# drdeford/FlipComplexityEmpirical

Measured on AMD Instinct MI355X. Metric: flip steps/sec (whole node), 100×100 grid k=4 batched chains; % HBM peak, higher is better.
Workload: dtype int32

## Files before the change

flipcomplexityempirical_amd/csrc/fw_grid16.hip:

```cpp
#include <hip/hip_runtime.h>

#include <cstdio>
#include <cstdlib>

#include <algorithm>

#include "fw_device.h"

#ifdef FW_STAMPS
__device__ unsigned long long g_stamps[16];
__device__ unsigned long long g_unit_t[2 * 65536];
__device__ unsigned long long g_unit_hw[65536];
#define UNIT_TIME(u, e)                                                         \
  do {                                                                          \
    uint64_t t_;                                                                \
    asm volatile("s_memrealtime %0\n\ts_waitcnt lgkmcnt(0)" : "=s"(t_)::"memory"); \
    if (__lane_id() == 0 && (u) < 65536) {                                      \
      g_unit_t[2 * (u) + (e)] = t_;                                             \
      if ((e) == 0)                                                             \
        g_unit_hw[u] = (unsigned long long)__builtin_amdgcn_s_getreg((31 << 11) | 4) | \
                       ((unsigned long long)__builtin_amdgcn_s_getreg((31 << 11) | 20) << 32); \
    }                                                                           \
  } while (0)
#define STAMP_DECL uint64_t st_acc[16] = {}; uint64_t st_t0 = 0;
// ... 7 lines not shown
    st_t0 = st_t1;                                            \
  } while (0)
#define STAMP_FLUSH                                           \
  if (__lane_id() == 0)                                       \
    for (int i_ = 0; i_ < 16; ++i_) atomicAdd(&g_stamps[i_], (unsigned long long)st_acc[i_]);
#define STAMP_COUNT(i, v) st_acc[i] += (uint64_t)(v)
#else
#define STAMP_COUNT(i, v)
#define STAMP_DECL
#define STAMP(i)
#define STAMP_FLUSH
#define UNIT_TIME(u, e)
#endif

#include <cstddef>

static_assert(sizeof(fw_chain_stats) == 136, "fw_chain_stats layout");
static_assert(offsetof(fw_chain_stats, yields) == 88 && offsetof(fw_chain_stats, sum_invb) == 112 &&
                  offsetof(fw_chain_stats, cut) == 120 && offsetof(fw_chain_stats, npairs) == 128,
              "fw_chain_stats layout");

#define HIST_ADD(ptr, v) atomicAdd(ptr, v)

void* fw_grid16_pick_lean(int lb, int mode, int G);
void* fw_grid16_pick_w2(int mode, int G);

namespace {

constexpr int ROW = 16;
constexpr int MAX_NW = 4;
constexpr uint32_t SCR_BLOCK = 15;
constexpr int LDS_GUARD = 16;

struct Hood16 {
  int x;
  uint32_t lx;
  uint32_t bits;
  uint32_t cnt;
  bool has_v;
  int deg;
};

struct GDiv {
  uint32_t m, s;
  __device__ __forceinline__ int operator()(int x) const {
    return (int)(__umul24((uint32_t)x, m) >> s);
  }
};
// ... 74 lines not shown
__device__ __forceinline__ uint32_t bsum4(uint32_t v) {
  return (v & 0xFFu) + ((v >> 8) & 0xFFu) + ((v >> 16) & 0xFFu) + (v >> 24);
}

__device__ __forceinline__ uint32_t spread4(uint32_t u) {
  const uint32_t t = ((u << 12) | u) & 0x000F000Fu;
  return ((t << 6) | t) & 0x03030303u;
}
__device__ __forceinline__ uint32_t onehot4(uint32_t s) {
  return __builtin_amdgcn_perm(0u, 0x08040201u, s);
}
__device__ __forceinline__ uint32_t low_bytes(int t) {
  const uint32_t tc = (uint32_t)min(max(t, 0), 4);
  return tc == 4u ? 0xFFFFFFFFu : (1u << (8u * tc)) - 1u;
}
__device__ __forceinline__ uint32_t ne_bytes(uint32_t a, uint32_t b) {
  return ~((a & b) + 0x7F7F7F7Fu) & 0x80808080u;
}
__device__ __forceinline__ uint32_t byte_popc(uint32_t f) {
  const uint32_t t = f - ((f >> 1) & 0x55555555u);
  return (t & 0x33333333u) + ((t >> 2) & 0x33333333u);
}

template <int MODE, bool NEED_CD, bool BATCH = true>
__device__ __forceinline__ void weights4_swar(const LDS uint8_t* lab, int x0, int W, int H, int n,
                                              GDiv gd, uint32_t& w4, uint32_t& cd4) {
  w4 = 0;
  cd4 = 0;
  const int xs = x0 < n ? x0 : 0;
  const bool hasU = xs + 3 - W >= 0, hasD = xs + W < n;
  const LDS uint32_t* lw32 = reinterpret_cast<const LDS uint32_t*>(lab);
  const int xw[3] = {xs, hasU ? xs - W : xs, hasD ? xs + W : xs};
  uint32_t wlo[3], whi[3];
  int wbit[3];
#pragma unroll
  for (int t = 0; t < 3; ++t) {
    wbit[t] = (xw[t] - 1) * 2;
    const int wi = wbit[t] >> 5;
    wlo[t] = lw32[wi];
    whi[t] = lw32[wi + 1];
  }
  const int r0 = gd(x0);
  const int c0 = x0 - mulW(r0, W);
  const int tw = W - c0;
  const uint32_t t8 = (uint32_t)min(tw, 4) << 3;
  const uint32_t nxt = (uint32_t)(~0ull << t8);
  const uint32_t mN = low_bytes(n - x0);
  const uint32_t mU = r0 > 0 ? 0xFFFFFFFFu : nxt;
  const uint32_t mD = r0 < H - 2 ? 0xFFFFFFFFu : (r0 == H - 2 ? ~nxt : 0u);
  const uint32_t mL = ~((uint32_t)(0xFFull << t8) | (c0 == 0 ? 0xFFu : 0u));
  const uint32_t mR = ~(uint32_t)(0xFFull << (((uint32_t)min(tw, 5) << 3) - 8u));
  if constexpr (BATCH) __builtin_amdgcn_sched_barrier(0);
  uint32_t win[3];
#pragma unroll
  for (int t = 0; t < 3; ++t) {
    const int wi = wbit[t] >> 5;
    const uint64_t both = ((uint64_t)whi[t] << 32) | (wi >= 0 ? wlo[t] : 0u);
    win[t] = (uint32_t)(both >> (uint32_t)(wbit[t] - wi * 32)) & 0xFFFu;
  }
  const uint32_t own = win[0];
  const uint32_t up = hasU ? win[1] : 0u, dn = hasD ? win[2] : 0u;
  const uint32_t o_lo = onehot4(spread4(own)), o_hi = onehot4(spread4(own >> 8));
  const uint32_t L = o_lo;
  const uint32_t O = __builtin_amdgcn_alignbyte(o_hi, o_lo, 1);
  const uint32_t R = __builtin_amdgcn_alignbyte(o_hi, o_lo, 2);
  const uint32_t U = onehot4(spread4(up >> 2)), Dn = onehot4(spread4(dn >> 2));
  if constexpr (MODE != FW_PROPOSE_CUTEDGE) {
    const uint32_t bits = (U & mU) | (L & mL) | (R & mR) | (Dn & mD);
    w4 = byte_popc(bits & ~O & mN);
  }
  if constexpr (NEED_CD || MODE == FW_PROPOSE_CUTEDGE) {
    const uint32_t ne = (ne_bytes(U, O) & mU) >> 7, nl = (ne_bytes(L, O) & mL) >> 7,
                   nr = (ne_bytes(R, O) & mR) >> 7, nd = (ne_bytes(Dn, O) & mD) >> 7;
    cd4 = (ne + nl + nr + nd) & mN;
    if constexpr (MODE == FW_PROPOSE_CUTEDGE) w4 = cd4;
  }
}

template <int LB, int MODE, bool NEED_CD, bool BATCH = true>
__device__ __forceinline__ void weights4x(const LDS uint8_t* lab, int x0, int W, int H, int n,
                                          GDiv gd, uint32_t& w4, uint32_t& cd4) {
  if constexpr (LB == 2)
    weights4_swar<MODE, NEED_CD, BATCH>(lab, x0, W, H, n, gd, w4, cd4);
  else
    weights4<LB, MODE>(lab, x0, W, H, n, gd, w4, cd4);
}

__device__ __forceinline__ uint32_t bsum4m(uint32_t v) { return (v * 0x01010101u) >> 24; }


__device__ __forceinline__ int window_verdict8(uint64_t A, int q, int row, bool need, uint32_t& nflood) {
#ifdef FW_STAMPS
#define FLOOD_COUNT ++nflood
#else
#define FLOOD_COUNT
#endif
  constexpr uint64_t BORDER = 0x7Full | (0x7Full << 48) | 0x0001010101010101ull | 0x0040404040404040ull;
  const uint64_t src = A & ((1ull << 19) | (1ull << 26) | (1ull << 28) | (1ull << 35));
  const int sb = q == 0 ? 19 : q == 1 ? 26 : q == 2 ? 28 : 35;
  uint64_t x = (need && q < 4) ? src & (1ull << sb) : 0ull;
  if (x) {
    for (;;) {
      const uint64_t y = (x | (x << 1) | (x >> 1) | (x << 8) | (x >> 8)) & A;
      x = (y | (y << 1) | (y >> 1) | (y << 8) | (y >> 8)) & A;
      FLOOD_COUNT;
      if (x == y) break;
// ... 226 lines not shown
    lb = le;
    le = nl;
    rep = ballot(lane < m && (__ffsll((unsigned long long)cls) - 1) == lane);
    if (__popcll(rep) == 1) {
      verdict = 1;
      break;
    }
    const bool closed = lane < m && ((rep >> lane) & 1ull) && ((cls & pushed_src) == 0ull);
    if (ballot(closed)) {
      verdict = 0;
      break;
    }
  }
  bfs_deg += wave_sum(my_deg);
  for (int base = 0; base < nl; base += WAVE) {
    const int idx = base + lane;
    if (idx < nl) scr_clear(scr, (int)list_get(idx));
  }
  if (lane == 0) scr_clear(scr, v);
  lds_order();
  return verdict == 1;
}

template <int LB, int MODE, int PER, bool FULL, bool BIG, int R, bool W2 = false>
__device__ __forceinline__ void grid16_body(const FwRunParams& p) {
  static_assert(PER % 2 == 0, "group sums are read as u16 pairs");
  static_assert(R == 1 || R == 2 || R == 4, "rows per chain");
  static_assert(R == 1 || (!FULL && !BIG), "speculation: lean small-grid kernels only");
  constexpr int CPW = 4 / R;
  extern __shared__ __align__(16) uint8_t smem[];
  __shared__ int32_t s_lock;
  using P = PK<LB>;
  const int lane = __lane_id(), row = lane >> 4, q = lane & 15;
  const int sx = row & (R - 1);
  const int grp = row / R;
  const int gb = grp * R * ROW;
  const bool owner = sx == 0;
  const int wv = (int)(threadIdx.x >> 6);
  const int W = (int)in_vgpr((uint32_t)p.g.gw), H = (int)in_vgpr((uint32_t)p.g.gh);
  const int n = (int)in_vgpr((uint32_t)p.g.n);
  const int D = (int)in_vgpr((uint32_t)p.g.maxdeg), G = (int)in_vgpr((uint32_t)p.G);
  const int k = (int)in_vgpr((uint32_t)p.k);
  LDS uint8_t* const sm = (LDS uint8_t*)smem;
  LDS uint8_t* const lab = sm + LDS_GUARD + (wv * CPW + grp) * p.slot_stride;
  LDS uint32_t* const gsum = reinterpret_cast<LDS uint32_t*>(lab + p.off_gsum);
  LDS uint32_t* const ssum = reinterpret_cast<LDS uint32_t*>(lab + p.off_ssum);
  LDS uint32_t* const lvl1 = BIG ? ssum : gsum;
  LDS uint8_t* const scr = sm + p.off_scr;
// ... 66 lines not shown
      LDS u32x4* dst = reinterpret_cast<LDS u32x4*>(lab);
      const int nv = cached ? p.lab_copy16 : p.lab_bytes / 16;
      for (int i = sx * ROW + ql; i < nv; i += R * ROW) dst[i] = src[i];
    }
    int32_t pops = ql < k ? (int32_t)p.pops[(size_t)cc * k + ql] : 0;
    double thr_l = FULL && ql < 2 * D + 1 ? p.thr[(size_t)cc * p.thr_stride + ql] : 0.0;
    uint64_t thr53_l = ql < 2 * D + 1 ? p.thr53[(size_t)cc * p.thr_stride + ql] : 0ull;
    fw_chain_stats* stp = p.stats + cc;
    const uint64_t acc0 = FULL && p.sched ? stp->accepts : 0ull;
    auto sched_row = [&](uint64_t nacc) {
      const int64_t t = (int64_t)(acc0 + nacc) + 1 - p.sched_t0;
      const int64_t r = t < 0 ? 0 : (t >= p.sched_rows ? p.sched_rows - 1 : t);
      if (q < 2 * D + 1) {
        thr_l = p.sched[r * (2 * D + 1) + q];
        thr53_l = p.sched53[r * (2 * D + 1) + q];
      }
    };
    if (FULL && p.sched) sched_row(0);
    uint64_t att0 = stp->attempts;
    const bool first = has && !stp->stuck && stp->yields == 0 && att0 == 0;
    uint32_t n_att = 0;
    const uint64_t yields0 = stp->yields;
    int32_t stuck = has ? stp->stuck : 1;
    int64_t sum_cut = stp->sum_cut, sum_bnodes = stp->sum_bnodes;
    double sum_invb = stp->sum_invb;
    const bool waits_on = FULL && p.wsamp != nullptr;
    double wsum = waits_on ? p.wsamp[2 * (size_t)cc] : 0.0;
    double wcur = waits_on ? p.wsamp[2 * (size_t)cc + 1] : 0.0;
    uint32_t n_steps = 0, n_acc = 0, n_popf = 0, n_conf = 0, n_sdeg = 0, n_adeg = 0, n_bchg = 0;
    uint32_t retries = 0;
    uint64_t n_bfs = 0, n_bfsn = 0, n_bfsd = 0;
    uint32_t bpos_w = ROW * R;
    Pend pend = maps_on ? pend_load(p, cc) : Pend{-1, 0, 0u};
    int32_t bcnt = rule == FW_ACCEPT_BOUNDARY && ql < k ? p.bcnt[(size_t)cc * k + ql] : 0;
    lds_order();

    int32_t cut, bnodes, npairs;
    {
      uint32_t cut2 = 0, bn = 0, np = 0;
      for (int t2 = 0; t2 < (cached ? 0 : GW); ++t2) {
        uint32_t tot[2];
#pragma unroll
        for (int h = 0; h < 2; ++h) {
          uint32_t w4, cd4;
          weights4x<LB, MODE, true>(lab, (2 * t2 + h) * 64 + q * 4, W, H, n, gd, w4, cd4);
          const uint32_t ws = bsum4m(w4);
          cut2 += bsum4m(cd4);
          bn += ((cd4 & 0xFFu) != 0) + ((cd4 & 0xFF00u) != 0) + ((cd4 & 0xFF0000u) != 0) +
                ((cd4 & 0xFF000000u) != 0);
          np += ws;
          tot[h] = row_sum(ws);
        }
        if (q == 0 && has) gsum[t2] = tot[0] | (tot[1] << 16);
      }
      if constexpr (BIG) {
        for (int t2 = GW + q; t2 < SG * 8; t2 += ROW)
          if (has) gsum[t2] = 0u;
        lds_order();
        for (int w2 = q; w2 < 8 * PER; w2 += ROW) {
          uint32_t s2[2] = {0u, 0u};
#pragma unroll
          for (int h = 0; h < 2; ++h) {
            const int sg = 2 * w2 + h;
            if (sg < SG)
              for (int i = 0; i < 8; ++i) {
                const uint32_t g2 = gsum[sg * 8 + i];
                s2[h] += (g2 & 0xFFFFu) + (g2 >> 16);
              }
// ... 22 lines not shown
      int f = -1, sc = -1;
      for (int b0 = 0; b0 < RN; b0 += ROW) {
        const int r = b0 + q;
        const int ri = r < RN ? r : 0;
        uint32_t m = rowbits(ballot(r < RN && P::get(lab, p.ring_u[ri]) != P::get(lab, p.ring_w[ri])),
                             row);
        if (m && f < 0) {
          f = b0 + __ffs(m) - 1;
          m &= m - 1;
        }
        if (m && sc < 0) sc = b0 + __ffs(m) - 1;
      }
      return sc >= 0 ? f * RN + sc : RN * RN;
    };
    int32_t rpair = RN && has ? ring_pair() : 0;
    uint32_t rrun = 0;

    uint32_t hc0 = 0, hc1 = 0, hb0 = 0, hb1 = 0;
    int32_t base_c = max(0, cut - 16), base_b = max(0, bnodes - 16);
    auto observe = [&](bool on) {
      if (!on) return;
      if (FULL) rrun += 1;
      if (waits_on) wsum += wcur;
      sum_cut += cut;
      sum_bnodes += bnodes;
      sum_invb += invb;
      int ic = cut - base_c;
      if (ic < 0 || ic >= 2 * ROW) {
        if (hc0) HIST_ADD(p.hist_cut + base_c + q, (unsigned long long)hc0);
        if (hc1) HIST_ADD(p.hist_cut + base_c + ROW + q, (unsigned long long)hc1);
        hc0 = hc1 = 0;
        base_c = max(0, cut - ROW);
        ic = cut - base_c;
      }
      hc0 += ic == q;
      hc1 += ic == q + ROW;
      int ib = bnodes - base_b;
      if (ib < 0 || ib >= 2 * ROW) {
        if (hb0) HIST_ADD(p.hist_b + base_b + q, (unsigned long long)hb0);
        if (hb1) HIST_ADD(p.hist_b + base_b + ROW + q, (unsigned long long)hb1);
        hb0 = hb1 = 0;
        base_b = max(0, bnodes - ROW);
        ib = bnodes - base_b;
      }
      hb0 += ib == q;
      hb1 += ib == q + ROW;
    };
    if (waits_on && first) wcur = wait_draw(p.seed, FW_WAIT_T0, gid, p.wlp[bnodes]);
    observe(first && owner);

    U4 pb = {0u, 0u, 0u, 0u};
    int bpos = ROW;

    const bool unit_pop = !FULL || p.g.pop == nullptr;
    const uint32_t psh = (uint32_t)p.prio_shift;
    const uint32_t pstep = ustep >= (2u << psh) ? ustep >> psh : 2u;
    uint32_t pnext = pstep, plev = 0;
    if (psh == 3u && (__builtin_amdgcn_s_getreg((3 << 11) | 4) & 1u) == 0u) plev = 1;
    if (plev == 0) __builtin_amdgcn_s_setprio(3);
    else __builtin_amdgcn_s_setprio(2);
    for (;;) {
      STAMP(-1);
      if (!stuck && (retries >= (uint32_t)p.max_retries || npairs == 0)) stuck = 1;
      const bool act = has && !stuck && n_steps < ustep;
      if (ballot(act) == 0ull) break;
      if (rfl(n_steps) >= pnext) {
        pnext += pstep;
        plev = (plev + 1u) & 3u;
        if (plev == 0) __builtin_amdgcn_s_setprio(3);
        else if (plev == 1) __builtin_amdgcn_s_setprio(2);
        else if (plev == 2) __builtin_amdgcn_s_setprio(1);
        else __builtin_amdgcn_s_setprio(0);
      }

      U4 x;
      if constexpr (R == 1) {
        if (bpos == ROW) {
          if (n_sdeg >= p.fold_at) {
            if (q == 0 && has) {
              stp->pop_fail += n_popf;
              stp->contig_fail += n_conf;
              stp->sum_deg += n_sdeg;
            }
            att0 += n_att;
            n_att = n_popf = n_conf = n_sdeg = 0;
          }
          const uint64_t t = att0 + (uint64_t)(n_att + (uint32_t)q);
          pb = philox((uint32_t)t, (uint32_t)(t >> 32), (uint32_t)gid, (uint32_t)(gid >> 32),
                      in_vgpr(key0), in_vgpr(key1));
          bpos = 0;
        }
        x = U4{row_first(pb.x0), row_first(pb.x1), row_first(pb.x2), row_first(pb.x3)};
        pb = U4{row_shl1(pb.x0), row_shl1(pb.x1), row_shl1(pb.x2), row_shl1(pb.x3)};
        ++bpos;
        n_att += act ? 1u : 0u;
      } else {
        if (bpos_w > (uint32_t)(ROW * R - R)) {
          if (4u * n_att >= p.fold_at) {
            const uint32_t f0 = grp_sum<R>(n_popf, gb, q), f1 = grp_sum<R>(n_conf, gb, q);
            const uint32_t f2 = grp_sum<R>(n_sdeg, gb, q);
            if (q == 0 && owner && has) {
              stp->pop_fail += f0;
              stp->contig_fail += f1;
              stp->sum_deg += f2;
            }
            att0 += n_att;
            n_att = n_popf = n_conf = n_sdeg = 0;
          }
          const uint64_t t = att0 + (uint64_t)(n_att + (uint32_t)(sx * ROW + q));
          pb = philox((uint32_t)t, (uint32_t)(t >> 32), (uint32_t)gid, (uint32_t)(gid >> 32),
                      in_vgpr(key0), in_vgpr(key1));
          bpos_w = 0;
        }
        const int srcl = gb + (int)bpos_w + sx;
        x = U4{lane_read(pb.x0, srcl), lane_read(pb.x1, srcl), lane_read(pb.x2, srcl),
               lane_read(pb.x3, srcl)};
      }
      const uint32_t r = scale64(x.x0, x.x1, (uint32_t)(npairs > 0 ? npairs : 1));

      STAMP(0);
      uint32_t w2[PER / 2];
      uint32_t s = 0;
#pragma unroll
      for (int t = 0; t < PER / 2; ++t) {
        w2[t] = lvl1[q * (PER / 2) + t];
        s += (w2[t] & 0xFFFFu) + (w2[t] >> 16);
      }
      uint32_t pp[PER / 2];
      {
        uint32_t base = 0;
#pragma unroll
        for (int t = 0; t < PER / 2; ++t) {
          pp[t] = __umul24(base, 0x10001u) + (w2[t] + (w2[t] << 16));
          base = pp[t] >> 16;
        }
      }
      const uint32_t incl = row_scan(s);
      const uint32_t rb1 = rowbits(ballot(incl > r), row);
      const int Lw = __ffs(rb1) - 1;
      const uint32_t rl = r - (incl - s);
      typedef uint16_t u16x2 __attribute__((ext_vector_type(2)));
      const u16x2 rl2 = __builtin_bit_cast(u16x2, __umul24(rl & 0xFFFFu, 0x10001u));
      u16x2 mn = {0xFFFFu, 0xFFFFu}, wraps = {0u, 0u};
#pragma unroll
      for (int t = 0; t < PER / 2; ++t) {
        const u16x2 e = rl2 - __builtin_bit_cast(u16x2, pp[t]);
        mn = __builtin_elementwise_min(mn, e);
        wraps += e >> (uint16_t)15;
      }
      const uint32_t rem = min(rl, (uint32_t)min(mn.x, mn.y));
// ... 3 lines not shown
      int gi;
      uint32_t r1;
      uint32_t rbg = 1u;
      if constexpr (BIG) {
        const int sgi = min((int)(pk1 >> 16), SG - 1);
        const uint32_t r1s = pk1 & 0xFFFFu;
        const uint32_t g2 = gsum[sgi * 8 + (q >> 1)];
        const uint32_t gv = (q & 1) ? (g2 >> 16) : (g2 & 0xFFFFu);
        const uint32_t incg = row_scan(gv);
        rbg = rowbits(ballot(incg > r1s), row);
        const int Lg = __ffs(rbg) - 1;
        const uint32_t pkg =
            row_pick(((uint32_t)(sgi * 16 + q) << 16) | ((r1s - (incg - gv)) & 0xFFFFu), Lg, q);
        gi = min((int)(pkg >> 16), G - 1);
        r1 = pkg & 0xFFFFu;
      } else {
        gi = min((int)(pk1 >> 16), G - 1);
        r1 = pk1 & 0xFFFFu;
      }

      STAMP(1);
      const int x0 = gi * 64 + q * 4;
      uint32_t w4, cd4;
      weights4x<LB, MODE, false, !W2>(lab, x0, W, H, n, gd, w4, cd4);
      const uint32_t pref1 = w4 + (w4 << 8);
      const uint32_t pref = pref1 + (pref1 << 16);
      const uint32_t ws = pref >> 24;
      const uint32_t incl2 = row_scan(ws);
      const uint32_t rb2 = rowbits(ballot(incl2 > r1), row);
      const int L2 = __ffs(rb2) - 1;
      const uint32_t r2 = min(r1 - (incl2 - ws), 127u);
      const uint32_t gt = ((pref | 0x80808080u) - __builtin_amdgcn_perm(0u, r2 + 1u, 0u)) & 0x80808080u;
      const int t2 = gt ? (__ffs(gt) - 1) >> 3 : 3;
      const uint32_t bef2 = t2 ? (pref >> (8 * t2 - 8)) & 0xFFu : 0u;
      const uint32_t pk2 = row_pick(((uint32_t)(q * 4 + t2) << 16) | ((r2 - bef2) & 0xFFFFu), L2, q);
      const int v = min(gi * 64 + (int)(pk2 >> 16), n - 1);
      const uint32_t j = pk2 & 0xFFFFu;
      if (R == 1 && act && (rb1 == 0 || rb2 == 0 || rbg == 0)) stuck = 2;
      const bool go = act && rb1 != 0 && rb2 != 0 && rbg != 0;

      STAMP(2);
      int vr, vc;
      divmod(v, vr, vc);
      const int dv = (vr > 0) + (vc > 0) + (vc < W - 1) + (vr < H - 1);
      Hood16 h;
      h.x = -1;
      h.lx = NOLAB;
// ... 290 lines not shown
          }
        }
        if (sx < (int)cons) {
          n_sdeg += (uint32_t)dv;
          if (!pop_ok) n_popf += 1;
          else if (!contig) n_conf += 1;
          n_bfs += it_bfs;
          n_bfsn += it_bfsn;
          n_bfsd += it_bfsd;
        }
        n_steps = ns;
        retries = rt;
        n_att += cons;
        bpos_w += cons;
        const bool commit_me = sx == fpos;
        if (commit_me) {
          n_acc += 1;
          n_adeg += (uint32_t)dv;
          n_bchg += (uint32_t)(plus + minus);
          if (q == 0) P::axor(lab, v, a ^ d);
          if (mine && wn != wo) lds_add(gsum + (h.x >> 7), (wn - wo) << (16 * ((h.x >> 6) & 1)));
        }
        lds_order();
        uint32_t dl = commit_me && mine ? wn - wo : 0u;
        dl += (uint32_t)__builtin_amdgcn_update_dpp(0, (int)dl, 0x111, 0xF, 0xF, true);
        dl += (uint32_t)__builtin_amdgcn_update_dpp(0, (int)dl, 0x112, 0xF, 0xF, true);
        dl += (uint32_t)__builtin_amdgcn_update_dpp(0, (int)dl, 0x114, 0xF, 0xF, true);
        const int dnp = (int)(uint32_t)__builtin_amdgcn_update_dpp(0, (int)dl, 0x154, 0xF, 0xF, false);
        const int fsrc = gb + (fpos < 0 ? 0 : fpos) * ROW + q;
        const uint32_t pk = (uint32_t)(dcut + 8) | ((uint32_t)plus << 4) | ((uint32_t)minus << 8) |
                            (a << 12) | (d << 16) | ((uint32_t)(dnp + 64) << 20);
        const uint32_t pkf = lane_read(pk, fsrc);
        const uint64_t ib = (uint64_t)__double_as_longlong(invb_new);
        const uint32_t ibl = lane_read((uint32_t)ib, fsrc), ibh = lane_read((uint32_t)(ib >> 32), fsrc);
        for (uint32_t i = 0; i < kold; ++i) observe(owner);
        if (fpos >= 0) {
          npairs += (int)((pkf >> 20) & 127u) - 64;
          cut += (int)(pkf & 15u) - 8;
          bnodes += (int)((pkf >> 4) & 15u) - (int)((pkf >> 8) & 15u);
          invb = __longlong_as_double((long long)(((uint64_t)ibh << 32) | ibl));
          if ((uint32_t)q == ((pkf >> 12) & 15u)) pops -= 1;
          if ((uint32_t)q == ((pkf >> 16) & 15u)) pops += 1;
          observe(owner);
        }
        STAMP(5);
        continue;
// ... 24 lines not shown
        p.trace[(size_t)c * p.steps + n_steps] = accepted ? v * 64 + (int)d : -1;
      n_steps += valid ? 1u : 0u;
      if (maps_on && accepted) {
        const int64_t t = (int64_t)(yields0 + (n_steps - 1u) + (first ? 1u : 0u));
        if (q >= 1 && q <= 4 && h.x >= 0 && (h.lx == a || h.lx == d)) {
          const int e = q == 1   ? grid_eid_down(vr - 1, vc, W, H)
                        : q == 2 ? grid_eid_right(vr, vc - 1, W, H)
                        : q == 3 ? grid_eid_right(vr, vc, W, H)
                                 : grid_eid_down(vr, vc, W, H);
          map_edge(p, c, e, h.lx == a, t);
        }
        if (q == 0) map_run_end(p, c, pend, t);
        pend = Pend{v, (int32_t)d, (uint32_t)t};
      }

      if (accepted) {
        if (q == 0) P::axor(lab, v, a ^ d);
        if (mine && wn != wo) {
          lds_add(gsum + (h.x >> 7), (wn - wo) << (16 * ((h.x >> 6) & 1)));
          if (BIG) lds_add(ssum + (h.x >> 11), (wn - wo) << (16 * ((h.x >> 10) & 1)));
        }
      }
      lds_order();
      uint32_t dl = accepted && mine ? wn - wo : 0u;
      dl += (uint32_t)__builtin_amdgcn_update_dpp(0, (int)dl, 0x111, 0xF, 0xF, true);
      dl += (uint32_t)__builtin_amdgcn_update_dpp(0, (int)dl, 0x112, 0xF, 0xF, true);
      dl += (uint32_t)__builtin_amdgcn_update_dpp(0, (int)dl, 0x114, 0xF, 0xF, true);
      const int dnp = (int)(uint32_t)__builtin_amdgcn_update_dpp(0, (int)dl, 0x154, 0xF, 0xF, false);
      if (FULL && RN && accepted && p.ring_node[v]) {
        const int32_t np2 = ring_pair();
        if (np2 != rpair) {
          if (q == 0 && rrun) atomicAdd(p.hist_ring + rpair, (unsigned long long)rrun);
          rrun = 0;
          rpair = np2;
        }
      }
      STAMP(9);
      asm volatile("" ::"v"(invb_new));
      invb = accepted ? invb_new : invb;
      if (accepted) {
        n_acc += 1;
        if (FULL && p.sched) sched_row(n_acc);
        n_adeg += (uint32_t)dv;
        npairs += dnp;
        cut += dcut;
        bnodes += plus - minus;
// ... 35 lines not shown
      for (int i = qw; i < p.lab_copy16; i += ROW) dst[i] = src[i];
      if (qw < k) p.pops[(size_t)c * k + qw] = (int64_t)pops;
      if (qw < k && rule == FW_ACCEPT_BOUNDARY) p.bcnt[(size_t)c * k + qw] = bcnt;
      if (q == 0 && maps_on) pend_store(p, c, pend);
      if (q == 0 && waits_on) {
        p.wsamp[2 * (size_t)c] = wsum;
        p.wsamp[2 * (size_t)c + 1] = wcur;
      }
      if (q <= 8) {
        int qr = qw;
        if constexpr (!OPQ) asm volatile("" : "+v"(qr));
        uint64_t* rec = reinterpret_cast<uint64_t*>(stp) + 2 * qr;
        const uint64_t o0 = rec[0];
        const uint64_t o1 = qr < 8 ? rec[1] : 0ull;
        const uint64_t yinc = (uint64_t)n_steps + (first ? 1u : 0u);
        uint64_t w0, w1;
        switch (q) {
          case 0: w0 = att0 + n_att; w1 = o1 + n_steps; break;
          case 1: w0 = o0 + n_acc; w1 = o1 + n_popf; break;
          case 2: w0 = o0 + n_conf; w1 = o1 + n_bfs; break;
          case 3: w0 = o0 + n_bfsn; w1 = o1 + n_bfsd; break;
          case 4: w0 = o0 + n_sdeg; w1 = o1 + n_adeg; break;
          case 5: w0 = o0 + n_bchg; w1 = o1 + yinc; break;
          case 6: w0 = (uint64_t)sum_cut; w1 = (uint64_t)sum_bnodes; break;
          case 7:
            w0 = (uint64_t)__double_as_longlong(sum_invb);
            w1 = (uint64_t)(uint32_t)cut | ((uint64_t)(uint32_t)bnodes << 32);
            break;
          default: w0 = (uint64_t)(uint32_t)npairs | ((uint64_t)(uint32_t)stuck << 32); w1 = 0;
        }
        if (qr < 8) {
          typedef uint64_t u64x2 __attribute__((ext_vector_type(2)));
          *reinterpret_cast<u64x2*>(rec) = u64x2{w0, w1};
        } else {
          rec[0] = w0;
        }
      }
    }
    lds_order();
    UNIT_TIME(u, 1);
    if (seg + 1 < p.slices) {
      __builtin_amdgcn_fence(__ATOMIC_RELEASE, "agent");
      __hip_atomic_store(p.seg_done + quad, seg + 1, __ATOMIC_RELAXED, __HIP_MEMORY_SCOPE_AGENT);
    }
  }
  STAMP_FLUSH
}

template <int LB, int MODE, int PER, bool FULL, bool BIG>
__global__ __launch_bounds__(64 * MAX_NW) __attribute__((amdgpu_waves_per_eu(3))) void fw_grid16_kernel(FwRunParams p) {
  static_assert(!FULL, "FULL instantiations: fw_grid16_full_kernel");
  grid16_body<LB, MODE, PER, FULL, BIG, 1>(p);
}
template <int LB, int MODE, int PER, bool FULL, bool BIG>
__global__ __launch_bounds__(64 * MAX_NW) void fw_grid16_full_kernel(FwRunParams p) {
  grid16_body<LB, MODE, PER, true, BIG, 1>(p);
}
template <int LB, int MODE, int PER>
__global__ __launch_bounds__(64 * MAX_NW) void fw_grid16_w2_kernel(FwRunParams p) {
  grid16_body<LB, MODE, PER, false, false, 1, true>(p);
}

#ifndef FW_SPEC_WPE
#define FW_SPEC_WPE 3
#endif
template <int LB, int MODE, int PER, int R>
__global__ __launch_bounds__(64 * MAX_NW) __attribute__((amdgpu_waves_per_eu(FW_SPEC_WPE))) void
fw_grid16_spec_kernel(FwRunParams p) {
  grid16_body<LB, MODE, PER, false, false, R>(p);
}

int per16(int G) { return G <= 16 * 2 ? 2 : G <= 16 * 4 ? 4 : G <= 16 * 10 ? 10 : 16; }
int per16_big(int G) { return (G + 15) / 16 <= 32 ? 2 : 4; }
bool is_big(int G) { return G > 16 * 16; }

template <int LB, int MODE, int PER, bool FULL, bool BIG>
void* k16() {
  if constexpr (FULL)
    return reinterpret_cast<void*>(&fw_grid16_full_kernel<LB, MODE, PER, true, BIG>);
  else
    return reinterpret_cast<void*>(&fw_grid16_kernel<LB, MODE, PER, false, BIG>);
}

template <int LB, int MODE>
void* pick16_small_lean(int G) {
  switch (per16(G)) {
    case 2: return k16<LB, MODE, 2, false, false>();
    case 4: return k16<LB, MODE, 4, false, false>();
    case 10: return k16<LB, MODE, 10, false, false>();
    default: return k16<LB, MODE, 16, false, false>();
  }
}

template <int LB, int MODE, bool FULL>
void* pick16(int G) {
  if (is_big(G)) {
    if constexpr (LB == 4) {
      return nullptr;
    } else {
      return per16_big(G) == 2
                 ? k16<LB, MODE, 2, FULL, true>()
                 : k16<LB, MODE, 4, FULL, true>();
    }
  }
  if constexpr (LB == 3) {
    return nullptr;
  } else if constexpr (FULL) {
    switch (per16(G)) {
      case 2: return k16<LB, MODE, 2, true, false>();
      case 4: return k16<LB, MODE, 4, true, false>();
      case 10: return k16<LB, MODE, 10, true, false>();
      default: return k16<LB, MODE, 16, true, false>();
    }
  } else {
#if defined(FW_STAMPS)
    return pick16_small_lean<LB, MODE>(G);
#else
    return fw_grid16_pick_lean(LB, MODE, G);
#endif
  }
}

template <int MODE>
void* pick16_w2(int G) {
  if (is_big(G)) return nullptr;
  switch (per16(G)) {
    case 2: return reinterpret_cast<void*>(&fw_grid16_w2_kernel<2, MODE, 2>);
    case 4: return reinterpret_cast<void*>(&fw_grid16_w2_kernel<2, MODE, 4>);
    case 10: return reinterpret_cast<void*>(&fw_grid16_w2_kernel<2, MODE, 10>);
    default: return reinterpret_cast<void*>(&fw_grid16_w2_kernel<2, MODE, 16>);
  }
}

template <int LB, int MODE, int R>
void* pick16_spec(int G) {
  if (is_big(G) || LB == 3) return nullptr;
  switch (per16(G)) {
    case 2: return reinterpret_cast<void*>(&fw_grid16_spec_kernel<LB, MODE, 2, R>);
    case 4: return reinterpret_cast<void*>(&fw_grid16_spec_kernel<LB, MODE, 4, R>);
    case 10: return reinterpret_cast<void*>(&fw_grid16_spec_kernel<LB, MODE, 10, R>);
    default: return reinterpret_cast<void*>(&fw_grid16_spec_kernel<LB, MODE, 16, R>);
  }
}

template <int R>
void* pick16_spec_mode(const FwRunParams& p) {
  const bool cut = p.mode == FW_PROPOSE_CUTEDGE;
  if (p.lb == 2)
    return cut ? pick16_spec<2, FW_PROPOSE_CUTEDGE, R>(p.G) : pick16_spec<2, FW_PROPOSE_PAIRS, R>(p.G);
  if (p.lb == 4)
    return cut ? pick16_spec<4, FW_PROPOSE_CUTEDGE, R>(p.G) : pick16_spec<4, FW_PROPOSE_PAIRS, R>(p.G);
  return nullptr;
}

template <bool FULL>
void* pick16_mode(const FwRunParams& p) {
  const bool cut = p.mode == FW_PROPOSE_CUTEDGE;
  if (p.lb == 2)
    return cut ? pick16<2, FW_PROPOSE_CUTEDGE, FULL>(p.G) : pick16<2, FW_PROPOSE_PAIRS, FULL>(p.G);
  if (p.lb == 3)
    return cut ? pick16<3, FW_PROPOSE_CUTEDGE, FULL>(p.G) : pick16<3, FW_PROPOSE_PAIRS, FULL>(p.G);
  return cut ? pick16<4, FW_PROPOSE_CUTEDGE, FULL>(p.G) : pick16<4, FW_PROPOSE_PAIRS, FULL>(p.G);
}

int round16i(int x) { return (x + 15) / 16 * 16; }

}

#if defined(FW_G16_W2_TU) || defined(FW_STAMPS)
void* fw_grid16_pick_w2(int mode, int G) {
  return mode == FW_PROPOSE_CUTEDGE ? pick16_w2<FW_PROPOSE_CUTEDGE>(G) : pick16_w2<FW_PROPOSE_PAIRS>(G);
}
#endif
#if defined(FW_G16_LEAN_TU) || defined(FW_STAMPS)
void* fw_grid16_pick_lean(int lb, int mode, int G) {
  const bool cut = mode == FW_PROPOSE_CUTEDGE;
  if (is_big(G)) return nullptr;
  if (lb == 2) return cut ? pick16_small_lean<2, FW_PROPOSE_CUTEDGE>(G) : pick16_small_lean<2, FW_PROPOSE_PAIRS>(G);
  if (lb == 4) return cut ? pick16_small_lean<4, FW_PROPOSE_CUTEDGE>(G) : pick16_small_lean<4, FW_PROPOSE_PAIRS>(G);
  return nullptr;
}
#endif
#if !defined(FW_G16_W2_TU) && !defined(FW_G16_LEAN_TU)

#ifdef FW_STAMPS
extern "C" int fw_debug_unit_times(unsigned long long* out, int n) {
  if (n > 65536) return -1;
  if (hipMemcpyFromSymbol(out, HIP_SYMBOL(g_unit_t), sizeof(unsigned long long) * 2 * n) !=
      hipSuccess)
    return -1;
  return hipMemcpyFromSymbol(out + 2 * n, HIP_SYMBOL(g_unit_hw), sizeof(unsigned long long) * n) ==
                 hipSuccess ? 0 : -1;
}
extern "C" int fw_debug_stamps(unsigned long long* out, int reset) {
  if (hipMemcpyFromSymbol(out, HIP_SYMBOL(g_stamps), sizeof(unsigned long long) * 16) != hipSuccess)
    return -1;
  if (reset) {
    unsigned long long z[16] = {};
    if (hipMemcpyToSymbol(HIP_SYMBOL(g_stamps), z, sizeof z) != hipSuccess) return -1;
  }
  return 0;
}
// ... 2 lines not shown
int big_max_k() {
  const char* e = getenv("FLIPWALK_BIG_K8");
  return e && e[0] == '1' ? 8 : 4;
}

bool fw_grid16_candidate(int gw, int maxdeg, int G, int k, int64_t total_pop) {
  return gw >= 4 && maxdeg == 4 && total_pop < (1ll << 31) - 1 &&
         ((G <= 16 * 16 && k <= 15) || (G <= 64 * 16 && k <= big_max_k()));
}

int fw_grid16_lb(int G, int k) { return k <= 4 ? 2 : (is_big(G) ? 3 : 4); }

static bool grid16_full(const FwRunParams& p) {
  return p.m_acc != nullptr || p.accept != FW_ACCEPT_CUT || p.sched != nullptr || p.ring_n > 0 ||
         p.trace != nullptr || p.g.pop != nullptr || p.wsamp != nullptr;
}

int fw_grid16_launch_rows(const FwRunParams& p) { return grid16_full(p) ? 1 : p.spec; }

int fw_grid16_launch_nw(const FwRunParams& p) { return p.nw * fw_grid16_launch_rows(p) / p.spec; }

static void* grid16_fn_w2(const FwRunParams& p) {
  if (p.lb != 2) return nullptr;
  return fw_grid16_pick_w2(p.mode, p.G);
}

static void* grid16_fn_r(const FwRunParams& p, bool full, int R) {
  if (full) return pick16_mode<true>(p);
  if (R == 1 && p.w2) {
    void* f = grid16_fn_w2(p);
    if (f) return f;
  }
  if (R == 2) return pick16_spec_mode<2>(p);
  if (R == 4) return pick16_spec_mode<4>(p);
  return pick16_mode<false>(p);
}

void* fw_grid16_fn(const FwRunParams& p) {
  return grid16_fn_r(p, grid16_full(p), fw_grid16_launch_rows(p));
}

int fw_grid16_plan(FwRunParams& p, int device, int* grid) {
  p.w2 = 0;
  const bool big = is_big(p.G);
  const int gbytes = big ? round16i((p.G + 15) / 16 * 16 * 2) : 4 * 8 * per16(p.G);
  const int sbytes = big ? 4 * 8 * per16_big(p.G) : 0;
  const int slot = round16i(p.lab_bytes) + gbytes + sbytes;
// ... 103 lines not shown
        }
      }
      if (w_nw) {
        p.w2 = 1;
        best_nw = w_nw;
        best_blocks = w_blocks;
        best_lds = w_lds;
      }
    }
  }
  p.spec = best_r;
  p.nw = best_nw;
  const int cpw = 4 / best_r;
  p.off_scr = LDS_GUARD + cpw * best_nw * stride;
  p.off_list16 = p.off_scr + p.scr_bytes;
  p.lds16 = best_lds;
  for (int f = 0; f < 2; ++f) {
    void* fn = grid16_fn_r(p, f == 1, f == 1 ? 1 : best_r);
    if (fn && hipFuncSetAttribute(fn, hipFuncAttributeMaxDynamicSharedMemorySize, best_lds) != hipSuccess)
      return -1;
  }
  const char* verbose = getenv("FLIPWALK_VERBOSE");
  if (verbose && verbose[0] == '1')
    fprintf(stderr, "flipwalk: grid kernel %s%s, %d-bit labels, %d row(s) per chain, LDS %d B per "
            "workgroup of %d waves, %d workgroups (%d chains) per CU\n",
            is_big(p.G) ? "large-grid plan" : "small-grid plan", p.w2 ? " (W2 register budget)" : "",
            p.lb, best_r, best_lds, best_nw, best_blocks, best_blocks * best_nw * cpw);
  const long long per_wg = (long long)cpw * best_nw;
  long long gsz = (long long)best_blocks * prop.multiProcessorCount;
  const long long need = (p.n_chains + per_wg - 1) / per_wg;
  if (gsz > need) gsz = need;
  *grid = (int)(gsz < 1 ? 1 : gsz);
  return 0;
}

int fw_grid16_launch(const FwRunParams& p, int grid, void* stream) {
  void* args[] = {const_cast<FwRunParams*>(&p)};
  void* fn = fw_grid16_fn(p);
  if (!fn) return (int)hipErrorInvalidDeviceFunction;
  hipError_t e = hipFuncSetAttribute(fn, hipFuncAttributeMaxDynamicSharedMemorySize, p.lds16);
  if (e != hipSuccess) return (int)e;
  return (int)hipLaunchKernel(fn, dim3(grid), dim3(64 * fw_grid16_launch_nw(p)), args,
                              (size_t)p.lds16, (hipStream_t)stream);
}
#endif
```

Before: 4.205 billion.

## Specialize SWAR edge masks for width-multiple-of-4 grids and cache level-1 sums

Adds a W4 template specialization for grids whose width is a multiple of 4, so each 4-cell group never straddles a row and the boundary masks reduce to simple selects. It also keeps the per-lane level-1 group sums in registers, re-reading them from LDS only after commits instead of on every step. Per-step cut and boundary-node accumulators become 32-bit counters folded into the stats on the same schedule as the other counters, replacing 64-bit adds. This brings more kernel instantiations and code size, and the wider fold condition and the assumption that cached sums stay valid add correctness risk.

Measured after the change: 4.262 billion, median of 6. +1.4%, better.

```diff
diff --git a/flipcomplexityempirical_amd/csrc/fw_grid16.hip b/flipcomplexityempirical_amd/csrc/fw_grid16.hip
--- a/flipcomplexityempirical_amd/csrc/fw_grid16.hip
+++ b/flipcomplexityempirical_amd/csrc/fw_grid16.hip
@@ -53,8 +53,8 @@
 
 #define HIST_ADD(ptr, v) atomicAdd(ptr, v)
 
-void* fw_grid16_pick_lean(int lb, int mode, int G);
-void* fw_grid16_pick_w2(int mode, int G);
+void* fw_grid16_pick_lean(int lb, int mode, int G, bool w4);
+void* fw_grid16_pick_w2(int mode, int G, bool w4);
 
 namespace {
 
@@ -175,7 +175,7 @@
   return (t & 0x33333333u) + ((t >> 2) & 0x33333333u);
 }
 
-template <int MODE, bool NEED_CD, bool BATCH = true>
+template <int MODE, bool NEED_CD, bool BATCH = true, bool W4 = false>
 __device__ __forceinline__ void weights4_swar(const LDS uint8_t* lab, int x0, int W, int H, int n,
                                               GDiv gd, uint32_t& w4, uint32_t& cd4) {
   w4 = 0;
@@ -196,13 +196,22 @@
   const int r0 = gd(x0);
   const int c0 = x0 - mulW(r0, W);
   const int tw = W - c0;
-  const uint32_t t8 = (uint32_t)min(tw, 4) << 3;
-  const uint32_t nxt = (uint32_t)(~0ull << t8);
-  const uint32_t mN = low_bytes(n - x0);
-  const uint32_t mU = r0 > 0 ? 0xFFFFFFFFu : nxt;
-  const uint32_t mD = r0 < H - 2 ? 0xFFFFFFFFu : (r0 == H - 2 ? ~nxt : 0u);
-  const uint32_t mL = ~((uint32_t)(0xFFull << t8) | (c0 == 0 ? 0xFFu : 0u));
-  const uint32_t mR = ~(uint32_t)(0xFFull << (((uint32_t)min(tw, 5) << 3) - 8u));
+  uint32_t mN, mU, mD, mL, mR;
+  if constexpr (W4) {
+    mN = x0 < n ? 0xFFFFFFFFu : 0u;
+    mU = r0 > 0 ? 0xFFFFFFFFu : 0u;
+    mD = r0 < H - 1 ? 0xFFFFFFFFu : 0u;
+    mL = c0 == 0 ? 0xFFFFFF00u : 0xFFFFFFFFu;
+    mR = tw == 4 ? 0x00FFFFFFu : 0xFFFFFFFFu;
+  } else {
+    const uint32_t t8 = (uint32_t)min(tw, 4) << 3;
+    const uint32_t nxt = (uint32_t)(~0ull << t8);
+    mN = low_bytes(n - x0);
+    mU = r0 > 0 ? 0xFFFFFFFFu : nxt;
+    mD = r0 < H - 2 ? 0xFFFFFFFFu : (r0 == H - 2 ? ~nxt : 0u);
+    mL = ~((uint32_t)(0xFFull << t8) | (c0 == 0 ? 0xFFu : 0u));
+    mR = ~(uint32_t)(0xFFull << (((uint32_t)min(tw, 5) << 3) - 8u));
+  }
   if constexpr (BATCH) __builtin_amdgcn_sched_barrier(0);
   uint32_t win[3];
 #pragma unroll
@@ -230,11 +239,11 @@
   }
 }
 
-template <int LB, int MODE, bool NEED_CD, bool BATCH = true>
+template <int LB, int MODE, bool NEED_CD, bool BATCH = true, bool W4 = false>
 __device__ __forceinline__ void weights4x(const LDS uint8_t* lab, int x0, int W, int H, int n,
                                           GDiv gd, uint32_t& w4, uint32_t& cd4) {
   if constexpr (LB == 2)
-    weights4_swar<MODE, NEED_CD, BATCH>(lab, x0, W, H, n, gd, w4, cd4);
+    weights4_swar<MODE, NEED_CD, BATCH, W4>(lab, x0, W, H, n, gd, w4, cd4);
   else
     weights4<LB, MODE>(lab, x0, W, H, n, gd, w4, cd4);
 }
@@ -507,8 +516,9 @@
   return verdict == 1;
 }
 
-template <int LB, int MODE, int PER, bool FULL, bool BIG, int R, bool W2 = false>
+template <int LB, int MODE, int PER, bool FULL, bool BIG, int R, bool W2 = false, bool W4 = false>
 __device__ __forceinline__ void grid16_body(const FwRunParams& p) {
+  static_assert(!W4 || LB == 2, "the width flag belongs to the SWAR weights");
   static_assert(PER % 2 == 0, "group sums are read as u16 pairs");
   static_assert(R == 1 || R == 2 || R == 4, "rows per chain");
   static_assert(R == 1 || (!FULL && !BIG), "speculation: lean small-grid kernels only");
@@ -621,7 +631,7 @@
     uint32_t n_att = 0;
     const uint64_t yields0 = stp->yields;
     int32_t stuck = has ? stp->stuck : 1;
-    int64_t sum_cut = stp->sum_cut, sum_bnodes = stp->sum_bnodes;
+    uint32_t s_cut = 0, s_bn = 0;
     double sum_invb = stp->sum_invb;
     const bool waits_on = FULL && p.wsamp != nullptr;
     double wsum = waits_on ? p.wsamp[2 * (size_t)cc] : 0.0;
@@ -642,7 +652,7 @@
 #pragma unroll
         for (int h = 0; h < 2; ++h) {
           uint32_t w4, cd4;
-          weights4x<LB, MODE, true>(lab, (2 * t2 + h) * 64 + q * 4, W, H, n, gd, w4, cd4);
+          weights4x<LB, MODE, true, true, W4>(lab, (2 * t2 + h) * 64 + q * 4, W, H, n, gd, w4, cd4);
           const uint32_t ws = bsum4m(w4);
           cut2 += bsum4m(cd4);
           bn += ((cd4 & 0xFFu) != 0) + ((cd4 & 0xFF00u) != 0) + ((cd4 & 0xFF0000u) != 0) +
@@ -711,8 +721,8 @@
       if (!on) return;
       if (FULL) rrun += 1;
       if (waits_on) wsum += wcur;
-      sum_cut += cut;
-      sum_bnodes += bnodes;
+      s_cut += (uint32_t)cut;
+      s_bn += (uint32_t)bnodes;
       sum_invb += invb;
       int ic = cut - base_c;
       if (ic < 0 || ic >= 2 * ROW) {
@@ -740,6 +750,12 @@
 
     U4 pb = {0u, 0u, 0u, 0u};
     int bpos = ROW;
+    uint32_t w2[PER / 2];
+    auto read_lvl1 = [&]() {
+#pragma unroll
+      for (int t = 0; t < PER / 2; ++t) w2[t] = lvl1[q * (PER / 2) + t];
+    };
+    read_lvl1();
 
     const bool unit_pop = !FULL || p.g.pop == nullptr;
     const uint32_t psh = (uint32_t)p.prio_shift;
@@ -765,14 +781,17 @@
       U4 x;
       if constexpr (R == 1) {
         if (bpos == ROW) {
-          if (n_sdeg >= p.fold_at) {
+          if (n_sdeg >= p.fold_at || (s_cut | s_bn) >= p.fold_at) {
             if (q == 0 && has) {
               stp->pop_fail += n_popf;
               stp->contig_fail += n_conf;
               stp->sum_deg += n_sdeg;
+              stp->sum_cut += s_cut;
+              stp->sum_bnodes += s_bn;
             }
             att0 += n_att;
             n_att = n_popf = n_conf = n_sdeg = 0;
+            s_cut = s_bn = 0;
           }
           const uint64_t t = att0 + (uint64_t)(n_att + (uint32_t)q);
           pb = philox((uint32_t)t, (uint32_t)(t >> 32), (uint32_t)gid, (uint32_t)(gid >> 32),
@@ -785,16 +804,20 @@
         n_att += act ? 1u : 0u;
       } else {
         if (bpos_w > (uint32_t)(ROW * R - R)) {
-          if (4u * n_att >= p.fold_at) {
+          const uint32_t s_any = lane_read(s_cut | s_bn, gb + q);
+          if (4u * n_att >= p.fold_at || s_any >= p.fold_at) {
             const uint32_t f0 = grp_sum<R>(n_popf, gb, q), f1 = grp_sum<R>(n_conf, gb, q);
             const uint32_t f2 = grp_sum<R>(n_sdeg, gb, q);
             if (q == 0 && owner && has) {
               stp->pop_fail += f0;
               stp->contig_fail += f1;
               stp->sum_deg += f2;
+              stp->sum_cut += s_cut;
+              stp->sum_bnodes += s_bn;
             }
             att0 += n_att;
             n_att = n_popf = n_conf = n_sdeg = 0;
+            s_cut = s_bn = 0;
           }
           const uint64_t t = att0 + (uint64_t)(n_att + (uint32_t)(sx * ROW + q));
           pb = philox((uint32_t)t, (uint32_t)(t >> 32), (uint32_t)gid, (uint32_t)(gid >> 32),
@@ -808,13 +831,9 @@
       const uint32_t r = scale64(x.x0, x.x1, (uint32_t)(npairs > 0 ? npairs : 1));
 
       STAMP(0);
-      uint32_t w2[PER / 2];
       uint32_t s = 0;
 #pragma unroll
-      for (int t = 0; t < PER / 2; ++t) {
-        w2[t] = lvl1[q * (PER / 2) + t];
-        s += (w2[t] & 0xFFFFu) + (w2[t] >> 16);
-      }
+      for (int t = 0; t < PER / 2; ++t) s += (w2[t] & 0xFFFFu) + (w2[t] >> 16);
       uint32_t pp[PER / 2];
       {
         uint32_t base = 0;
@@ -864,7 +883,7 @@
       STAMP(1);
       const int x0 = gi * 64 + q * 4;
       uint32_t w4, cd4;
-      weights4x<LB, MODE, false, !W2>(lab, x0, W, H, n, gd, w4, cd4);
+      weights4x<LB, MODE, false, !W2, W4>(lab, x0, W, H, n, gd, w4, cd4);
       const uint32_t pref1 = w4 + (w4 << 8);
       const uint32_t pref = pref1 + (pref1 << 16);
       const uint32_t ws = pref >> 24;
@@ -1201,6 +1220,7 @@
           if (mine && wn != wo) lds_add(gsum + (h.x >> 7), (wn - wo) << (16 * ((h.x >> 6) & 1)));
         }
         lds_order();
+        read_lvl1();
         uint32_t dl = commit_me && mine ? wn - wo : 0u;
         dl += (uint32_t)__builtin_amdgcn_update_dpp(0, (int)dl, 0x111, 0xF, 0xF, true);
         dl += (uint32_t)__builtin_amdgcn_update_dpp(0, (int)dl, 0x112, 0xF, 0xF, true);
@@ -1271,6 +1291,7 @@
         }
       }
       lds_order();
+      read_lvl1();
       uint32_t dl = accepted && mine ? wn - wo : 0u;
       dl += (uint32_t)__builtin_amdgcn_update_dpp(0, (int)dl, 0x111, 0xF, 0xF, true);
       dl += (uint32_t)__builtin_amdgcn_update_dpp(0, (int)dl, 0x112, 0xF, 0xF, true);
@@ -1352,7 +1373,7 @@
           case 3: w0 = o0 + n_bfsn; w1 = o1 + n_bfsd; break;
           case 4: w0 = o0 + n_sdeg; w1 = o1 + n_adeg; break;
           case 5: w0 = o0 + n_bchg; w1 = o1 + yinc; break;
-          case 6: w0 = (uint64_t)sum_cut; w1 = (uint64_t)sum_bnodes; break;
+          case 6: w0 = o0 + s_cut; w1 = o1 + s_bn; break;
           case 7:
             w0 = (uint64_t)__double_as_longlong(sum_invb);
             w1 = (uint64_t)(uint32_t)cut | ((uint64_t)(uint32_t)bnodes << 32);
@@ -1377,18 +1398,18 @@
   STAMP_FLUSH
 }
 
-template <int LB, int MODE, int PER, bool FULL, bool BIG>
+template <int LB, int MODE, int PER, bool FULL, bool BIG, bool W4 = false>
 __global__ __launch_bounds__(64 * MAX_NW) __attribute__((amdgpu_waves_per_eu(3))) void fw_grid16_kernel(FwRunParams p) {
   static_assert(!FULL, "FULL instantiations: fw_grid16_full_kernel");
-  grid16_body<LB, MODE, PER, FULL, BIG, 1>(p);
+  grid16_body<LB, MODE, PER, FULL, BIG, 1, false, W4>(p);
 }
 template <int LB, int MODE, int PER, bool FULL, bool BIG>
 __global__ __launch_bounds__(64 * MAX_NW) void fw_grid16_full_kernel(FwRunParams p) {
   grid16_body<LB, MODE, PER, true, BIG, 1>(p);
 }
-template <int LB, int MODE, int PER>
+template <int LB, int MODE, int PER, bool W4>
 __global__ __launch_bounds__(64 * MAX_NW) void fw_grid16_w2_kernel(FwRunParams p) {
-  grid16_body<LB, MODE, PER, false, false, 1, true>(p);
+  grid16_body<LB, MODE, PER, false, false, 1, true, W4>(p);
 }
 
 #ifndef FW_SPEC_WPE
@@ -1404,26 +1425,33 @@
 int per16_big(int G) { return (G + 15) / 16 <= 32 ? 2 : 4; }
 bool is_big(int G) { return G > 16 * 16; }
 
-template <int LB, int MODE, int PER, bool FULL, bool BIG>
+template <int LB, int MODE, int PER, bool FULL, bool BIG, bool W4 = false>
 void* k16() {
   if constexpr (FULL)
     return reinterpret_cast<void*>(&fw_grid16_full_kernel<LB, MODE, PER, true, BIG>);
   else
-    return reinterpret_cast<void*>(&fw_grid16_kernel<LB, MODE, PER, false, BIG>);
-}
-
+    return reinterpret_cast<void*>(&fw_grid16_kernel<LB, MODE, PER, false, BIG, W4>);
+}
+
+template <int LB, int MODE, bool W4>
+void* pick16_small_lean_w(int G) {
+  switch (per16(G)) {
+    case 2: return k16<LB, MODE, 2, false, false, W4>();
+    case 4: return k16<LB, MODE, 4, false, false, W4>();
+    case 10: return k16<LB, MODE, 10, false, false, W4>();
+    default: return k16<LB, MODE, 16, false, false, W4>();
+  }
+}
 template <int LB, int MODE>
-void* pick16_small_lean(int G) {
-  switch (per16(G)) {
-    case 2: return k16<LB, MODE, 2, false, false>();
-    case 4: return k16<LB, MODE, 4, false, false>();
-    case 10: return k16<LB, MODE, 10, false, false>();
-    default: return k16<LB, MODE, 16, false, false>();
-  }
+void* pick16_small_lean(int G, bool w4) {
+  if constexpr (LB == 2) {
+    if (w4) return pick16_small_lean_w<LB, MODE, true>(G);
+  }
+  return pick16_small_lean_w<LB, MODE, false>(G);
 }
 
 template <int LB, int MODE, bool FULL>
-void* pick16(int G) {
+void* pick16(int G, bool w4) {
   if (is_big(G)) {
     if constexpr (LB == 4) {
       return nullptr;
@@ -1444,21 +1472,21 @@
     }
   } else {
 #if defined(FW_STAMPS)
-    return pick16_small_lean<LB, MODE>(G);
+    return pick16_small_lean<LB, MODE>(G, w4);
 #else
-    return fw_grid16_pick_lean(LB, MODE, G);
+    return fw_grid16_pick_lean(LB, MODE, G, w4);
 #endif
   }
 }
 
-template <int MODE>
+template <int MODE, bool W4>
 void* pick16_w2(int G) {
   if (is_big(G)) return nullptr;
   switch (per16(G)) {
-    case 2: return reinterpret_cast<void*>(&fw_grid16_w2_kernel<2, MODE, 2>);
-    case 4: return reinterpret_cast<void*>(&fw_grid16_w2_kernel<2, MODE, 4>);
-    case 10: return reinterpret_cast<void*>(&fw_grid16_w2_kernel<2, MODE, 10>);
-    default: return reinterpret_cast<void*>(&fw_grid16_w2_kernel<2, MODE, 16>);
+    case 2: return reinterpret_cast<void*>(&fw_grid16_w2_kernel<2, MODE, 2, W4>);
+    case 4: return reinterpret_cast<void*>(&fw_grid16_w2_kernel<2, MODE, 4, W4>);
+    case 10: return reinterpret_cast<void*>(&fw_grid16_w2_kernel<2, MODE, 10, W4>);
+    default: return reinterpret_cast<void*>(&fw_grid16_w2_kernel<2, MODE, 16, W4>);
   }
 }
 
@@ -1486,11 +1514,12 @@
 template <bool FULL>
 void* pick16_mode(const FwRunParams& p) {
   const bool cut = p.mode == FW_PROPOSE_CUTEDGE;
+  const bool w4 = p.g.gw % 4 == 0;
   if (p.lb == 2)
-    return cut ? pick16<2, FW_PROPOSE_CUTEDGE, FULL>(p.G) : pick16<2, FW_PROPOSE_PAIRS, FULL>(p.G);
+    return cut ? pick16<2, FW_PROPOSE_CUTEDGE, FULL>(p.G, w4) : pick16<2, FW_PROPOSE_PAIRS, FULL>(p.G, w4);
   if (p.lb == 3)
-    return cut ? pick16<3, FW_PROPOSE_CUTEDGE, FULL>(p.G) : pick16<3, FW_PROPOSE_PAIRS, FULL>(p.G);
-  return cut ? pick16<4, FW_PROPOSE_CUTEDGE, FULL>(p.G) : pick16<4, FW_PROPOSE_PAIRS, FULL>(p.G);
+    return cut ? pick16<3, FW_PROPOSE_CUTEDGE, FULL>(p.G, w4) : pick16<3, FW_PROPOSE_PAIRS, FULL>(p.G, w4);
+  return cut ? pick16<4, FW_PROPOSE_CUTEDGE, FULL>(p.G, w4) : pick16<4, FW_PROPOSE_PAIRS, FULL>(p.G, w4);
 }
 
 int round16i(int x) { return (x + 15) / 16 * 16; }
@@ -1498,16 +1527,17 @@
 }
 
 #if defined(FW_G16_W2_TU) || defined(FW_STAMPS)
-void* fw_grid16_pick_w2(int mode, int G) {
-  return mode == FW_PROPOSE_CUTEDGE ? pick16_w2<FW_PROPOSE_CUTEDGE>(G) : pick16_w2<FW_PROPOSE_PAIRS>(G);
+void* fw_grid16_pick_w2(int mode, int G, bool w4) {
+  if (w4) return mode == FW_PROPOSE_CUTEDGE ? pick16_w2<FW_PROPOSE_CUTEDGE, true>(G) : pick16_w2<FW_PROPOSE_PAIRS, true>(G);
+  return mode == FW_PROPOSE_CUTEDGE ? pick16_w2<FW_PROPOSE_CUTEDGE, false>(G) : pick16_w2<FW_PROPOSE_PAIRS, false>(G);
 }
 #endif
 #if defined(FW_G16_LEAN_TU) || defined(FW_STAMPS)
-void* fw_grid16_pick_lean(int lb, int mode, int G) {
+void* fw_grid16_pick_lean(int lb, int mode, int G, bool w4) {
   const bool cut = mode == FW_PROPOSE_CUTEDGE;
   if (is_big(G)) return nullptr;
-  if (lb == 2) return cut ? pick16_small_lean<2, FW_PROPOSE_CUTEDGE>(G) : pick16_small_lean<2, FW_PROPOSE_PAIRS>(G);
-  if (lb == 4) return cut ? pick16_small_lean<4, FW_PROPOSE_CUTEDGE>(G) : pick16_small_lean<4, FW_PROPOSE_PAIRS>(G);
+  if (lb == 2) return cut ? pick16_small_lean<2, FW_PROPOSE_CUTEDGE>(G, w4) : pick16_small_lean<2, FW_PROPOSE_PAIRS>(G, w4);
+  if (lb == 4) return cut ? pick16_small_lean<4, FW_PROPOSE_CUTEDGE>(G, w4) : pick16_small_lean<4, FW_PROPOSE_PAIRS>(G, w4);
   return nullptr;
 }
 #endif
@@ -1556,7 +1586,7 @@
 
 static void* grid16_fn_w2(const FwRunParams& p) {
   if (p.lb != 2) return nullptr;
-  return fw_grid16_pick_w2(p.mode, p.G);
+  return fw_grid16_pick_w2(p.mode, p.G, p.g.gw % 4 == 0);
 }
 
 static void* grid16_fn_r(const FwRunParams& p, bool full, int R) {
@@ -1706,9 +1736,10 @@
   }
   const char* verbose = getenv("FLIPWALK_VERBOSE");
   if (verbose && verbose[0] == '1')
-    fprintf(stderr, "flipwalk: grid kernel %s%s, %d-bit labels, %d row(s) per chain, LDS %d B per "
+    fprintf(stderr, "flipwalk: grid kernel %s%s%s, %d-bit labels, %d row(s) per chain, LDS %d B per "
             "workgroup of %d waves, %d workgroups (%d chains) per CU\n",
             is_big(p.G) ? "large-grid plan" : "small-grid plan", p.w2 ? " (W2 register budget)" : "",
+            !big && !full && best_r == 1 && p.lb == 2 && p.g.gw % 4 == 0 ? " (W4 masks)" : "",
             p.lb, best_r, best_lds, best_nw, best_blocks, best_blocks * best_nw * cpw);
   const long long per_wg = (long long)cpw * best_nw;
   long long gsz = (long long)best_blocks * prop.multiProcessorCount;
```
